# Decade-qiu/Go2NetSpectra

Measured on AMD Instinct MI355X. Metric: Mpackets/s CMS update (device-resident, d=4 w=2^20) at 1/2/4/8 MI355X, higher is better.
Workload: dtype u32; 1 GPU; configs[1]: Count-Min d=4 w=2^20, 100M Zipf(1.1) 5-tuple headers in HBM per GPU, bit-exact counters; device_batch=100000000, key=5-tuple (37 B), parallelism=owner-key shards x1 (SrcIP slot; each GPU generates its shard of the stream), windows=steps use stream windows 0..619 (warmup first), none replayed

## Files before the change

go2netspectra_amd/csrc/gns_cm.hip:

```cpp
#include <algorithm>
#include <atomic>
#include <cstdlib>
#include <mutex>
#include <vector>

#include "gns_coldmask.cuh"
#include "gns_common.hpp"
#include "gns_ctl.cuh"
#include "gns_hh.hpp"
#include "gns_scan.cuh"
#include "gns_xcd.cuh"

namespace gns {

#ifndef GNS_TILE_BITS
#define GNS_TILE_BITS 12
#endif
#ifndef GNS_AP_THREADS
#define GNS_AP_THREADS 1024
#endif
#ifndef GNS_AP_ITEMS
#define GNS_AP_ITEMS 8
#endif
constexpr uint32_t kTileBitsMax = GNS_TILE_BITS;
// ... 2294 lines not shown
        uint32_t cum = 0, t = kHotKeys;
        for (int k = (int)kHotKeys - 1; k >= (int)(kHotMinBits * 8); k--) {
            cum += s_hh[r * kHotKeys + k];
            if (cum > kHot) break;
            t = (uint32_t)k;
        }
        const uint32_t tp = thr[r];
        hfull[r] = !(tp <= kHotKeys && t + 8u >= tp && hcn[r] <= kHotCand);
        thr[r] = t;
        hcnt[r] = 0;
    }
}

__global__ __launch_bounds__(256) void k_hot_collect(const uint32_t *C, CmGeom g, const uint32_t *thr,
                                                      uint32_t *hcnt, uint32_t *hot_ids, const uint32_t *hcand,
                                                      const uint32_t *hcn, const uint32_t *hfull) {
    const uint64_t stride = (uint64_t)gridDim.x * 256;
    for (uint32_t r = 0; r < g.d; r++) {
        const uint32_t *Cr = C + (uint64_t)r * g.w;
        const uint32_t t = thr[r];
        auto take = [&](uint32_t v, uint64_t c) {
            if (v >= (1u << (kHotMinBits - 1)) && hot_key(v) >= t) {
                const uint32_t q = atomicAdd(&hcnt[r], 1u);
                if (q < kHot) hot_ids[r * kHot + q] = (uint32_t)c;
            }
        };
        if (!hfull[r]) {
            const uint32_t nc = hcn[r];
            for (uint32_t i = blockIdx.x * 256 + threadIdx.x; i < nc; i += (uint32_t)stride) {
                const uint32_t c = hcand[(uint64_t)r * kHotCand + i];
                take(Cr[c], c);
            }
            continue;
        }
        if ((g.w & 3u) == 0) {
            const uint4 *C4 = reinterpret_cast<const uint4 *>(Cr);
            for (uint64_t c = (uint64_t)blockIdx.x * 256 + threadIdx.x; c < g.w / 4; c += stride) {
                const uint4 v = C4[c];
                take(v.x, 4 * c); take(v.y, 4 * c + 1); take(v.z, 4 * c + 2); take(v.w, 4 * c + 3);
            }
        } else {
            for (uint64_t c = (uint64_t)blockIdx.x * 256 + threadIdx.x; c < g.w; c += stride) take(Cr[c], c);
        }
    }
}

__global__ __launch_bounds__(1024) void k_hot_table(CmGeom g, uint32_t *hot_ids, uint32_t *hot_tab, uint32_t *hcn) {
    __shared__ uint32_t s_ids[8 * kHot];
    const uint32_t NS = g.d * kHot;
    for (uint32_t i = threadIdx.x; i < g.d * kHotTab; i += blockDim.x) hot_tab[i] = 0xFFFFFFFFu;
    if (threadIdx.x < g.d) hcn[threadIdx.x] = 0;
    for (uint32_t i = threadIdx.x; i < NS; i += blockDim.x) s_ids[i] = hot_ids[i];
    __syncthreads();
    for (uint32_t i = threadIdx.x; i < NS; i += blockDim.x) {
        const uint32_t r = i / kHot, h = i % kHot, b = s_ids[i];
        if (b == GNS_ID_NONE) continue;
        const uint32_t grp = hot_group(b);
        uint32_t j = 0;
        for (uint32_t h2 = 0; h2 < h; h2++) {
            const uint32_t b2 = s_ids[r * kHot + h2];
            j += (b2 != GNS_ID_NONE && hot_group(b2) == grp) ? 1u : 0u;
        }
        if (j < 4) hot_tab[r * kHotTab + grp * 4 + j] = b << kHotBits | h;
        else hot_ids[i] = GNS_ID_NONE;
    }
}

struct QueryArgs {
    const uint8_t *keys;
    uint32_t stride, aligned;
    uint64_t n;
    uint32_t K;
    CmGeom g;
    DictDev D;
    const uint32_t *C, *Fc, *S, *Fs;
    uint64_t *out;
};

__global__ __launch_bounds__(256) void k_query(QueryArgs a) {
    const uint64_t p = (uint64_t)blockIdx.x * 256 + threadIdx.x;
    if (p >= a.n) return;
    uint32_t kw[GNS_KWMAX];
    load_key_bytes<GNS_KWMAX>(a.keys + p * a.stride, a.K, a.aligned != 0, kw);
    const uint32_t id = dict_lookup(a.D, kw);
    uint32_t sz = 0, ct = 0;
    if (id != GNS_ID_NONE) {
        for (uint32_t rr = 0; rr < a.g.d; rr++) {
            const uint64_t c = (uint64_t)rr * a.g.w + row_index(a.g, mm3_n<GNS_KWMAX>(kw, a.K, a.g.seeds[rr]));
            if (a.Fs[c] == id) sz = max(sz, a.S[c]);
            if (a.Fc[c] == id) ct = max(ct, a.C[c]);
        }
    }
    a.out[p] = (uint64_t)ct << 32 | sz;
}

}

using namespace gns;

struct CmRead {
    HhScratch hh;
    uint8_t *qkeys = nullptr;
    uint64_t qkeys_n = 0;
    uint64_t *qout = nullptr;
    uint64_t qout_n = 0;
    void free_all() {
        hh.free_all();
        dfree(qkeys); dfree(qout);
        qkeys = nullptr; qout = nullptr;
        qkeys_n = qout_n = 0;
    }
};

struct gns_cm : FlowDict {
    int device = 0;
    hipStream_t stream = nullptr;
    CmGeom g{};
    KeyPlanN kp{};
    uint32_t K = 0, st = 0, ct = 0;
    uint32_t *C = nullptr, *S = nullptr, *Fc = nullptr, *Fs = nullptr;
    CmRead rd;
    std::atomic<uint32_t> period{0};
    std::mutex views_mu;
    std::vector<gns_cm_view *> views;
    uint32_t epoch = 0;
    uint64_t bmax = 0;
    uint32_t nblk_max = 0;
    uint32_t *keyid = nullptr, *idx = nullptr;
    uint64_t *cold = nullptr;
    uint64_t *pend[2] = {nullptr, nullptr};
    uint32_t *pcnt[2] = {nullptr, nullptr};
    uint32_t *ptotal = nullptr;
    uint32_t *hist = nullptr, *part = nullptr, *total = nullptr, *order = nullptr;
    uint64_t *entries = nullptr;
    uint32_t *rec_sizes = nullptr;
    uint64_t *ovf = nullptr;
    uint32_t *ovf_cnt = nullptr;
    uint64_t ovf_cap = 0;
    unsigned long long *stats = nullptr;
    uint32_t *hot_ids = nullptr;
    uint32_t *hot_tab = nullptr;
    long long *segtot = nullptr;
    uint32_t *hflag = nullptr, *hhist = nullptr, *hthr = nullptr, *hcnt = nullptr;
    uint32_t *hcand = nullptr, *hcn = nullptr;
    HotSum *hsum = nullptr;
    uint32_t *hflag2 = nullptr;
    uint32_t *work = nullptr;
    uint32_t ncu = 256;
    uint32_t *hres = nullptr;
    uint4 *chk = nullptr;
    bool warm = false;
    bool lds_ordered = false;
    uint32_t *h_pin = nullptr;
    HostStage stage[2];
    uint32_t *side_dev = nullptr;
    uint64_t side_n = 0;
    hipStream_t cstream = nullptr;
    hipEvent_t ev_copied[2] = {nullptr, nullptr}, ev_used[2] = {nullptr, nullptr};
    StageTimer timer;
};

struct gns_cm_view {
    gns_cm *cm = nullptr;
    hipStream_t stream = nullptr;
    hipEvent_t ready = nullptr;
    uint32_t *C = nullptr, *S = nullptr, *Fc = nullptr, *Fs = nullptr;
    CmRead rd;
    std::mutex mu;
    uint32_t period = ~0u;
};

struct ViewsQuiesced {
    std::unique_lock<std::mutex> reg;
    std::vector<std::unique_lock<std::mutex>> locks;
    explicit ViewsQuiesced(gns_cm *cm) : reg(cm->views_mu) {
        locks.reserve(cm->views.size());
        for (gns_cm_view *v : cm->views) locks.emplace_back(v->mu);
    }
};

namespace {

int cm_free_all(gns_cm *cm) {
    dfree(cm->C); dfree(cm->S); dfree(cm->Fc); dfree(cm->Fs); cm->rd.free_all();
    dfree(cm->keyid); dfree(cm->idx); dfree(cm->cold);
    dfree(cm->pend[0]); dfree(cm->pend[1]); dfree(cm->pcnt[0]); dfree(cm->pcnt[1]);
    dfree(cm->ptotal); dfree(cm->hist); dfree(cm->part); dfree(cm->total); dfree(cm->order);
    dfree(cm->entries); dfree(cm->rec_sizes); dfree(cm->ovf); dfree(cm->ovf_cnt); dfree(cm->stats);
    cm->stage[0].free_all(); cm->stage[1].free_all(); dfree(cm->side_dev);
    for (int i = 0; i < 2; i++) {
        if (cm->ev_copied[i]) (void)hipEventDestroy(cm->ev_copied[i]);
        if (cm->ev_used[i]) (void)hipEventDestroy(cm->ev_used[i]);
    }
    if (cm->cstream) (void)hipStreamDestroy(cm->cstream);
    dfree(cm->work);
    dfree(cm->hot_ids); dfree(cm->segtot); dfree(cm->hflag); dfree(cm->hhist); dfree(cm->hthr); dfree(cm->hcnt);
    dfree(cm->hcand); dfree(cm->hcn);
    dfree(cm->hsum); dfree(cm->hflag2); dfree(cm->hres); dfree(cm->chk); dfree(cm->hot_tab);
    cm->FlowDict::free_all();
    if (cm->h_pin) (void)hipHostFree(cm->h_pin);
    cm->timer.destroy();
    if (cm->stream) (void)hipStreamDestroy(cm->stream);
    return GNS_OK;
}

int cm_reset_state(gns_cm *cm) {
    const uint64_t cells = (uint64_t)cm->g.d * cm->g.w;
    GNS_HIP(hipMemsetAsync(cm->C, 0, cells * 4, cm->stream));
    GNS_HIP(hipMemsetAsync(cm->S, 0, cells * 4, cm->stream));
    GNS_HIP(hipMemsetAsync(cm->Fc, 0xFF, cells * 4, cm->stream));
    GNS_HIP(hipMemsetAsync(cm->Fs, 0xFF, cells * 4, cm->stream));
    GNS_HIP(hipMemsetAsync(cm->D.rec, 0, cm->dict_slots * cm->D.RW * 4, cm->stream));
    GNS_HIP(hipMemsetAsync(cm->hot_ids, 0xFF, (size_t)cm->g.d * kHot * 4, cm->stream));
    GNS_HIP(hipMemsetAsync(cm->hot_tab, 0xFF, (size_t)cm->g.d * kHotTab * 4, cm->stream));
    GNS_HIP(hipMemsetAsync(cm->hhist, 0, (size_t)cm->g.d * kHotKeys * 4, cm->stream));
    GNS_HIP(hipMemsetAsync(cm->hthr, 0xFF, 8 * 4, cm->stream));
    GNS_HIP(hipMemsetAsync(cm->hcn, 0, 16 * 4, cm->stream));
    GNS_HIP(hipMemsetAsync(cm->stats + 3, 0, 2 * sizeof(unsigned long long), cm->stream));
    GNS_HIP(hipMemsetAsync(cm->dctl, 0, 16, cm->stream));
    cm->claimed = 0;
    cm->full = false;
    cm->warm = false;
    return GNS_OK;
}

int cm_reclaim(gns_cm *cm, uint64_t min_slots = 0) {
    ViewsQuiesced q(cm);
    const uint64_t cells = (uint64_t)cm->g.d * cm->g.w;
    std::vector<DictIds> ids{{cm->Fc, cells}, {cm->Fs, cells}};
    const uint32_t period = cm->period.load();
    for (gns_cm_view *v : cm->views)
        if (v->period == period) { ids.push_back({v->Fc, cells}); ids.push_back({v->Fs, cells}); }
    return cm->reclaim(ids.data(), (int)ids.size(), min_slots, cm->stream);
}

template <int KIND, int MODE>
int cm_run_batch(gns_cm *cm, const InputDesc &in, uint64_t n) {
    if (n == 0) return GNS_OK;
    hipStream_t s = cm->stream;
    const uint32_t nblk = (uint32_t)((n + kChunk - 1) / kChunk);
    const CmGeom &g = cm->g;
    ScopedStage total_stage(cm->timer, 5);
    {
        CtlZero z;
        z.add(cm->ptotal, 8);
        z.add(cm->dctl + 1, 4);
        z.add(cm->hflag2, ((size_t)g.d * kHot + 2) * 4);
        z.add(cm->stats + 8, 8);
        z.add(cm->ovf_cnt, 4);
        z.add(cm->work, 4);
        z.add(cm->hflag, (size_t)g.d * kHot * 4);
        GNS_HIP(ctl_zero(z, s));
    }
    if (++cm->epoch == 0) cm->epoch = 1;
    {
        ExtractArgs a{};
        a.in = in; a.n = n; a.kp = cm->kp; a.g = g; a.D = cm->D; a.epoch = cm->epoch;
        a.keyid = cm->keyid; a.idx = cm->idx; a.cold = cm->cold; a.pend = cm->pend[0]; a.pend_cnt = cm->pcnt[0];
        a.pend_total = cm->ptotal; a.hist = cm->hist; a.nblk = nblk; a.hot_ids = cm->hot_ids;
        a.Fc = cm->Fc; a.Fs = cm->Fs; a.hsum = cm->hsum; a.hot_tab = cm->hot_tab;
        a.stats = cm->stats;
        ScopedStage st(cm->timer, 0);
        const size_t lds = extract_lds_bytes(g.nbins_all, g.d);
        if constexpr (KIND == IN_REC16) {
            if (lds > kExLdsSmall)
                hipLaunchKernelGGL((k_extract<KIND, MODE, 0, 0, 1024>), dim3(nblk), dim3(1024), lds, s, a);
            else
                hipLaunchKernelGGL((k_extract<KIND, MODE, 0, 0, 256>), dim3(nblk), dim3(kExThreads), lds, s, a);
        } else if (lds > kExLdsSmall) {
            if (cm->K == 37 && g.d == 8)
                hipLaunchKernelGGL((k_extract<KIND, MODE, 37, 8, kC5Threads>), dim3(nblk), dim3(kC5Threads), lds, s, a);
            else if (cm->K == 37)
                hipLaunchKernelGGL((k_extract<KIND, MODE, 37, 0, 1024>), dim3(nblk), dim3(1024), lds, s, a);
            else if (cm->K == 16)
                hipLaunchKernelGGL((k_extract<KIND, MODE, 16, 0, 1024>), dim3(nblk), dim3(1024), lds, s, a);
            else
                hipLaunchKernelGGL((k_extract<KIND, MODE, 0, 0, 1024>), dim3(nblk), dim3(1024), lds, s, a);
        } else if (cm->K == 37 && g.d == 4)
            hipLaunchKernelGGL((k_extract<KIND, MODE, 37, 4, 256>), dim3(nblk), dim3(kExThreads), lds, s, a);
        else if (cm->K == 37)
            hipLaunchKernelGGL((k_extract<KIND, MODE, 37, 0, 256>), dim3(nblk), dim3(kExThreads), lds, s, a);
        else if (cm->K == 16 && g.d == 4)
            hipLaunchKernelGGL((k_extract<KIND, MODE, 16, 4, 256>), dim3(nblk), dim3(kExThreads), lds, s, a);
        else if (cm->K == 16)
            hipLaunchKernelGGL((k_extract<KIND, MODE, 16, 0, 256>), dim3(nblk), dim3(kExThreads), lds, s, a);
        else
            hipLaunchKernelGGL((k_extract<KIND, MODE, 0, 0, 256>), dim3(nblk), dim3(kExThreads), lds, s, a);
        GNS_HIP(hipGetLastError());
    }
    int cur = 0;
    for (int round = 0;; round++) {
        if (round > 1) {
            CtlRead rd;
            rd.add(cm->ptotal + cur, 4, 0);
            rd.add(cm->stats + 3, 8, 2);
            rd.add(cm->dctl, 4, 4);
            if (round == 2) rd.add(cm->stats + 8, 8, 6);
            GNS_HIP(ctl_read(rd, cm->h_pin, s));
            GNS_HIP(hipStreamSynchronize(s));
            cm->claimed = cm->h_pin[4];
            if (round == 2) {
                const uint64_t big = (uint64_t)cm->h_pin[6] | (uint64_t)cm->h_pin[7] << 32;
                if (big * g.d > cm->ovf_cap) {
                    const uint64_t want = std::min<uint64_t>(std::max<uint64_t>(big * g.d + big * g.d / 4, kOvfCap), 1ull << 31);
                    dfree(cm->ovf);
                    cm->ovf = nullptr;
                    cm->ovf_cap = 0;
                    GNS_TRY(dalloc_t(&cm->ovf, want));
                    cm->ovf_cap = want;
                }
            }
            if (cm->h_pin[2] | cm->h_pin[3]) {
                set_error("flow dictionary full (%llu slots); raise max_flows",
                          (unsigned long long)cm->dict_slots);
                return GNS_E_FULL;
            }
            if (cm->h_pin[0] == 0) break;
        }
        if (round > 64) { set_error("dictionary resolve did not converge"); return GNS_E_FULL; }
        if (++cm->epoch == 0) cm->epoch = 1;
        ResolveArgs a{};
        a.in = in; a.n = n; a.kp = cm->kp; a.D = cm->D; a.epoch = cm->epoch; a.keyid = cm->keyid;
        a.pend_in = cm->pend[cur]; a.cnt_in = cm->pcnt[cur];
        a.pend_out = cm->pend[cur ^ 1]; a.cnt_out = cm->pcnt[cur ^ 1]; a.total_out = cm->ptotal + (cur ^ 1);
        a.total_in = cm->ptotal + cur;
        a.stats = cm->stats; a.g = g;
        ScopedStage st(cm->timer, 1);
        hipLaunchKernelGGL((k_resolve<KIND, MODE>), dim3(nblk), dim3(kExThreads), 0, s, a);
        GNS_HIP(hipGetLastError());
        cur ^= 1;
    }
    {
        ScopedStage st(cm->timer, 2);
        const uint32_t ngrp = (nblk + kTGrp - 1) / kTGrp;
        const dim3 g2((g.nbins_all + 255) / 256, ngrp);
        uint32_t *tot = cm->part + (size_t)ngrp * g.nbins_all;
        hipLaunchKernelGGL(k_tscan_part, g2, dim3(256), 0, s, cm->hist, nblk, g.nbins_all, cm->part);
        hipLaunchKernelGGL(k_tscan_mid, dim3((g.nbins_all + 255) / 256), dim3(256), 0, s, cm->part, ngrp, g.nbins_all, tot);
        hipLaunchKernelGGL(k_tscan_bins, dim3(1), dim3(1024), 0, s, tot, g.nbins_all, cm->total);
        hipLaunchKernelGGL(k_tscan_down, g2, dim3(256), 0, s, cm->hist, nblk, g.nbins_all, cm->part, tot);
        GNS_HIP(hipGetLastError());
    }
    {
        ScatterArgs a{};
        a.n = n; a.g = g; a.keyid = cm->keyid; a.idx = cm->idx; a.sizes = in.sizes;
        a.offsets = cm->hist; a.nblk = nblk; a.entries = cm->entries; a.ovf = cm->ovf; a.cold = cm->cold;
        a.ovf_cnt = cm->ovf_cnt; a.ovf_cap = (uint32_t)cm->ovf_cap; a.hot_ids = cm->hot_ids; a.stats = cm->stats;
        a.hot_mode = 0; a.hflag2 = cm->hflag2; a.hany = cm->hflag2 + g.d * kHot;
        ScopedStage st(cm->timer, 3);
        if (cm->lds_ordered && g.ntiles <= 256)
            hipLaunchKernelGGL((k_scatter_st<256, false>), dim3(nblk), dim3(kStThreads), 0, s, a);
        else if (cm->lds_ordered && g.ntiles <= 512)
            hipLaunchKernelGGL((k_scatter_st<512, true>), dim3(nblk), dim3(kStThreads), 0, s, a);
        else if (cm->lds_ordered)
            hipLaunchKernelGGL(k_scatter<1>, dim3(nblk), dim3(kScThreads), scatter_lds_bytes(g.ntiles + kHot, g.d), s, a);
        else
            hipLaunchKernelGGL(k_scatter<0>, dim3(nblk), dim3(kScThreads), scatter_lds_bytes(g.ntiles + kHot, g.d), s, a);
        GNS_HIP(hipGetLastError());
    }
    {
        const bool ordered = g.nbins <= 4096;
        if (ordered)
            hipLaunchKernelGGL(k_order, dim3(1), dim3(1024), 0, s, cm->hist, nblk, g.nbins, g.nbins_all,
                               cm->total, cm->order);
        ApplyArgs a{};
        a.stats = cm->stats;
        a.entries = cm->entries; a.offsets = cm->hist; a.nblk = nblk; a.nbins = g.nbins;
        a.total = cm->total; a.order = ordered ? cm->order : nullptr; a.ovf = cm->ovf; a.g = g;
        a.C = cm->C; a.Fc = cm->Fc; a.S = cm->S; a.Fs = cm->Fs; a.work = cm->work;
        ScopedStage st(cm->timer, 4);
        if (g.sub_bits) {
            const dim3 apg(std::min(g.nbins, cm->ncu));
            hipLaunchKernelGGL(k_apply_sparse, apg, dim3(kApThreads), 0, s, a);
        } else {
            const dim3 apg(std::min(g.nbins, cm->ncu * (kApThreads <= 512 ? 2u : 1u)));
            hipLaunchKernelGGL(k_apply, apg, dim3(kApThreads), 0, s, a);
        }
        GNS_HIP(hipGetLastError());
    }
    {
        HotArgs h{};
        h.entries = cm->entries; h.offsets = cm->hist; h.nblk = nblk; h.total = cm->total; h.ovf = cm->ovf;
        h.hot_ids = cm->hot_ids; h.g = g; h.C = cm->C; h.Fc = cm->Fc; h.S = cm->S; h.Fs = cm->Fs;
        h.segtot = cm->segtot; h.hflag = cm->hflag;
        h.hsum = cm->hsum; h.hflag2 = cm->hflag2; h.hany = cm->hflag2 + g.d * kHot; h.nchk = h.hany + 1;
        h.hres = cm->hres; h.chk = cm->chk; h.chk_cap = kChkCap;
        h.keyid = cm->keyid; h.idx = cm->idx; h.sizes = in.sizes; h.n = n;
        ScopedStage st(cm->timer, 6);
        hipLaunchKernelGGL(k_hot_decide, dim3(g.d * kHot), dim3(256), 0, s, h);
        hipLaunchKernelGGL(k_hot_blockcheck, dim3(kChkCap), dim3(256), 0, s, h);
        hipLaunchKernelGGL(k_hot_commit, dim3((g.d * kHot + 511) / 512), dim3(512), 0, s, h);
        {
            ScatterArgs a{};
            a.n = n; a.g = g; a.keyid = cm->keyid; a.idx = cm->idx; a.sizes = in.sizes;
            a.offsets = cm->hist; a.nblk = nblk; a.entries = cm->entries; a.ovf = cm->ovf;
            a.ovf_cnt = cm->ovf_cnt; a.ovf_cap = (uint32_t)cm->ovf_cap; a.hot_ids = cm->hot_ids; a.stats = cm->stats;
            a.hot_mode = 1; a.hflag2 = cm->hflag2; a.hany = h.hany;
            if (cm->lds_ordered)
                hipLaunchKernelGGL(k_scatter<1>, dim3(nblk), dim3(kScThreads), scatter_lds_bytes(g.ntiles + kHot, g.d), s, a);
            else
                hipLaunchKernelGGL(k_scatter<0>, dim3(nblk), dim3(kScThreads), scatter_lds_bytes(g.ntiles + kHot, g.d), s, a);
        }
        hipLaunchKernelGGL(k_hot_sum, dim3(1024), dim3(256), 0, s, h);
        hipLaunchKernelGGL(k_hot_verify, dim3(1024), dim3(256), 0, s, h);
        hipLaunchKernelGGL(k_hot_apply, dim3((g.d * kHot + 511) / 512), dim3(512), 0, s, h);
        hipLaunchKernelGGL(k_hot_fallback, dim3(g.d * kHot), dim3(64), 0, s, h);
        GNS_HIP(hipGetLastError());
    }
    {
        ScopedStage st(cm->timer, 7);
        const unsigned grid = (unsigned)std::min<uint64_t>(2048, ((uint64_t)g.w / 4 + 255) / 256 + 1);
        uint32_t *hcn = cm->hcn, *hfull = cm->hcn + 8;
        hipLaunchKernelGGL(k_hot_hist, dim3(std::min(grid, 512u)), dim3(256), 0, s, cm->C, g, cm->hhist, cm->hthr,
                           cm->hcand, hcn);
        hipLaunchKernelGGL(k_hot_pick, dim3(1), dim3(512), 0, s, cm->hhist, g, cm->hthr, cm->hcnt, cm->hot_ids, hcn,
                           hfull);
        hipLaunchKernelGGL(k_hot_collect, dim3(grid), dim3(256), 0, s, cm->C, g, cm->hthr, cm->hcnt, cm->hot_ids,
                           cm->hcand, hcn, hfull);
        hipLaunchKernelGGL(k_hot_table, dim3(1), dim3(1024), 0, s, g, cm->hot_ids, cm->hot_tab, hcn);
        GNS_HIP(hipGetLastError());
    }
    cm->warm = true;
    return GNS_OK;
}

template <int KIND>
int cm_batch(gns_cm *cm, const InputDesc &d, uint64_t m) {
    if constexpr (KIND == IN_KEYS) {
        return cm_run_batch<KIND, PLAN_SLICE0>(cm, d, m);
    } else {
        switch (plan_mode(cm->kp)) {
        case PLAN_SLICE0: return cm_run_batch<KIND, PLAN_SLICE0>(cm, d, m);
        case PLAN_SLICE4: return cm_run_batch<KIND, PLAN_SLICE4>(cm, d, m);
        default: return cm_run_batch<KIND, PLAN_GENERIC>(cm, d, m);
        }
    }
}

template <int KIND>
int cm_batch_recover(gns_cm *cm, const InputDesc &d, uint64_t m) {
    static const std::string piece = std::to_string(kChunk) + "-packet batch";
    const DictRecovery r{*cm, cm->stats, cm->stream, kChunk, piece.c_str(),
                         [cm](const InputDesc &pd, uint64_t pm) { return cm_batch<KIND>(cm, pd, pm); },
                         [cm](uint64_t min_slots) { return cm_reclaim(cm, min_slots); }};
    return r.batch(d, m, false);
}

__global__ __launch_bounds__(256) void k_rec_sizes(const uint32_t *rec16, uint64_t n, uint32_t *sizes) {
    const uint64_t i = (uint64_t)blockIdx.x * 256 + threadIdx.x;
    if (i < n) sizes[i] = rec16[i * 4 + 3] >> 16;
}

int stage_host_batch(gns_cm *cm, int b, const InputDesc &in, uint64_t off, uint64_t m, InputDesc &d) {
    if (!cm->cstream) {
        GNS_HIP(hipStreamCreateWithFlags(&cm->cstream, hipStreamNonBlocking));
        for (int i = 0; i < 2; i++) {
            GNS_HIP(hipEventCreateWithFlags(&cm->ev_copied[i], hipEventDisableTiming));
            GNS_HIP(hipEventCreateWithFlags(&cm->ev_used[i], hipEventDisableTiming));
        }
    }
    StageList l;
    d = advance(in, off);
    stage_input(l, d, m);
    if (in.rec_len) stage_add<uint32_t>(l, nullptr, m * 4, &d.sizes);
    HostStage &sg = cm->stage[b];
    if (sg.cap < HostStage::need(l)) GNS_HIP(hipEventSynchronize(cm->ev_used[b]));
    GNS_HIP(hipStreamWaitEvent(cm->cstream, cm->ev_used[b], 0));
    GNS_TRY(sg.copy(l, cm->cstream));
    if (in.rec_len) {
        hipLaunchKernelGGL(k_rec_sizes, dim3((unsigned)((m + 255) / 256)), dim3(256), 0, cm->cstream, d.rec16, m,
                           const_cast<uint32_t *>(d.sizes));
        GNS_HIP(hipGetLastError());
    }
    if (d.keys) d.aligned = (d.stride % 4 == 0 && d.stride >= ((cm->K + 3) & ~3u)) ? 1u : 0u;
    GNS_HIP(hipEventRecord(cm->ev_copied[b], cm->cstream));
    return GNS_OK;
}

template <int KIND>
int cm_insert(gns_cm *cm, InputDesc in, uint64_t n, gns_mem where) {
    GNS_TRY(set_device(cm->device));
    auto batch_len = [&](uint64_t off, bool warm) {
        const uint64_t m = std::min<uint64_t>(cm->bmax, n - off);
        return warm ? m : std::min<uint64_t>(m, std::max<uint64_t>(kChunk * 64, cm->bmax / 32));
    };
    if (where == GNS_MEM_DEVICE) {
        for (uint64_t off = 0, m = 0; off < n; off += m) {
            m = batch_len(off, cm->warm);
            InputDesc d = advance(in, off);
            if (in.rec_len) {
                if (!cm->rec_sizes) GNS_TRY(dalloc_t(&cm->rec_sizes, cm->bmax));
                hipLaunchKernelGGL(k_rec_sizes, dim3((unsigned)((m + 255) / 256)), dim3(256), 0, cm->stream, d.rec16, m,
                                   cm->rec_sizes);
                GNS_HIP(hipGetLastError());
                d.sizes = cm->rec_sizes;
            }
            GNS_TRY(cm_batch_recover<KIND>(cm, d, m));
        }
        return GNS_OK;
    }
    if (n == 0) return GNS_OK;
    bool warm = cm->warm;
    uint64_t off = 0, m = batch_len(0, warm);
    InputDesc d;
    GNS_TRY(stage_host_batch(cm, 0, in, 0, m, d));
    for (int b = 0;; b ^= 1) {
        const uint64_t noff = off + m;
        const uint64_t nm = noff < n ? batch_len(noff, true) : 0;
        InputDesc nd;
        if (nm) GNS_TRY(stage_host_batch(cm, b ^ 1, in, noff, nm, nd));
        GNS_HIP(hipStreamWaitEvent(cm->stream, cm->ev_copied[b], 0));
        const int rc = cm_batch_recover<KIND>(cm, d, m);
        GNS_HIP(hipEventRecord(cm->ev_used[b], cm->stream));
        if (rc != GNS_OK) {
            (void)hipStreamSynchronize(cm->cstream);
            return rc;
        }
        if (!nm) break;
        off = noff; m = nm; d = nd;
    }
    GNS_HIP(hipStreamSynchronize(cm->cstream));
    return GNS_OK;
}

}

extern "C" {

int gns_cm_create(const gns_cm_params *p, gns_cm **out) {
    if (!p || !out) { set_error("null argument"); return GNS_E_ARG; }
    *out = nullptr;
    GNS_TRY(check_device(p->device));
    gns_cm *cm = new gns_cm();
    cm->device = p->device;
    int rc = GNS_OK;
    do {
        if ((rc = set_device(cm->device)) != GNS_OK) break;
        CmGeom &g = cm->g;
        g.w = p->width ? p->width : (1u << 20);
        g.d = p->depth ? p->depth : 3u;
        cm->st = p->size_threshold ? p->size_threshold : 512u * 1024u;
        cm->ct = p->count_threshold ? p->count_threshold : 512u;
        if (g.d > 8) { set_error("depth %u > 8 not supported", g.d); rc = GNS_E_ARG; break; }
        if ((rc = make_plan(p->flow, p->key_bytes, &cm->kp)) != GNS_OK) break;
        cm->K = cm->kp.K;
        if (g.w >= (1u << (32 - kHotBits))) {
            set_error("width %u >= 2^%u is not supported", g.w, 32 - kHotBits); rc = GNS_E_RANGE; break;
        }
        if (p->bucket_lo == 0 && p->bucket_hi == 0) {
            g.blo = 0; g.bspan = g.w;
        } else if (p->bucket_lo < p->bucket_hi && p->bucket_hi <= g.w) {
            g.blo = p->bucket_lo; g.bspan = p->bucket_hi - p->bucket_lo;
        } else {
            set_error("bucket range [%u, %u) is not inside [0, %u)", p->bucket_lo, p->bucket_hi, g.w);
            rc = GNS_E_ARG; break;
        }
        g.pow2 = (g.w & (g.w - 1)) == 0;
        g.wmask = g.pow2 ? g.w - 1 : 0;
        uint32_t tb = kTileBitsMax;
        while (tb > 8 && (uint64_t)g.d * ((g.w + (1u << tb) - 1) >> tb) < 1024) tb--;
        g.tile_bits = tb;
        uint32_t sb = 0;
        auto bins_at = [&](uint32_t bits) { return (uint32_t)(((uint64_t)g.w + (1ull << bits) - 1) >> bits); };
        while (bins_at(tb + sb) > kMaxTilesPerRow || (uint64_t)g.d * bins_at(tb + sb) > kMaxBinsAll) sb++;
        if (tb + sb > kEntShift || sb > 4) {
            set_error("width %u with depth %u is too wide (max %u buckets per row at this depth)", g.w, g.d,
                      (uint32_t)std::min<uint64_t>(0xFFFFFFFFull, (uint64_t)std::min(kMaxTilesPerRow, kMaxBinsAll / g.d) << kEntShift));
            rc = GNS_E_RANGE;
            break;
        }
        g.sub_bits = sb;
        g.bin_bits = tb + sb;
        g.ntiles = bins_at(g.bin_bits);
        g.nbins = g.d * g.ntiles;
        g.nbins_all = g.nbins + g.d * kHot;
        g.nbits = ceil_log2(g.ntiles + kHot);
        if (p->seeds) for (uint32_t i = 0; i < g.d; i++) g.seeds[i] = p->seeds[i];
        else default_seeds(g.seeds, g.d);
        if (hipStreamCreateWithFlags(&cm->stream, hipStreamNonBlocking) != hipSuccess) {
            set_error("hipStreamCreate failed"); rc = GNS_E_HIP; break;
        }
        cm->timer.stream = cm->stream;
        {
            int ncu = 0;
            if (hipDeviceGetAttribute(&ncu, hipDeviceAttributeMultiprocessorCount, cm->device) == hipSuccess && ncu > 0)
                cm->ncu = (uint32_t)ncu;
        }
        const uint64_t cells = (uint64_t)g.d * g.w;
        if ((rc = dalloc_t(&cm->C, cells)) || (rc = dalloc_t(&cm->S, cells)) ||
            (rc = dalloc_t(&cm->Fc, cells)) || (rc = dalloc_t(&cm->Fs, cells)))
            break;
        const uint64_t mf = p->max_flows ? p->max_flows : (4ull << 20);
        uint64_t slots = 1;
        while (slots < 2 * mf) slots <<= 1;
        if (slots > kDictMaxSlots) { set_error("max_flows too large"); rc = GNS_E_ARG; break; }
        cm->dict_slots = slots;
        cm->max_flows = mf;
        cm->D.mask = (uint32_t)(slots - 1);
        cm->D.K = cm->K;
        cm->D.RW = dict_record_words_cm(cm->K, g.d);
        cm->D.bw = cm->D.RW >= 16 && 1 + (cm->K + 3) / 4 <= 12 ? 1u : 0u;
        cm->D.seed = 0x2545F491u;
        if ((rc = dalloc_t(&cm->D.rec, slots * cm->D.RW)) != GNS_OK) break;
        if ((rc = dalloc_t(&cm->dctl, 4)) != GNS_OK || (rc = dalloc_t(&cm->stats_bak, 3)) != GNS_OK) break;
        cm->D.ctl = cm->dctl;
        cm->limits();
        cm->bmax = p->batch_packets ? p->batch_packets : (16ull << 20);
        cm->bmax = ((cm->bmax + kChunk - 1) / kChunk) * kChunk;
        if (cm->bmax > (1ull << 31)) { set_error("batch_packets too large"); rc = GNS_E_ARG; break; }
        const uint64_t bcap = (((1ull << 31) / g.d) / kChunk) * kChunk;
        if (cm->bmax > bcap) cm->bmax = bcap;
        cm->nblk_max = (uint32_t)(cm->bmax / kChunk);
        const uint64_t nscan = ((uint64_t)(cm->nblk_max + kTGrp - 1) / kTGrp + 2) * g.nbins_all;
        if ((rc = dalloc_t(&cm->keyid, cm->bmax)) || (rc = dalloc_t(&cm->idx, cm->bmax * g.d)) ||
            (rc = dalloc_t(&cm->cold, cm->bmax / 64)) ||
            (rc = dalloc_t(&cm->pend[0], cm->bmax)) || (rc = dalloc_t(&cm->pend[1], cm->bmax)) ||
            (rc = dalloc_t(&cm->pcnt[0], cm->nblk_max)) || (rc = dalloc_t(&cm->pcnt[1], cm->nblk_max)) ||
            (rc = dalloc_t(&cm->ptotal, 2)) || (rc = dalloc_t(&cm->hist, (uint64_t)g.nbins_all * cm->nblk_max)) ||
            (rc = dalloc_t(&cm->part, nscan)) || (rc = dalloc_t(&cm->total, 1)) ||
            (rc = dalloc_t(&cm->order, g.nbins)) || (rc = dalloc_t(&cm->entries, cm->bmax * g.d)) ||
            (rc = dalloc_t(&cm->ovf, kOvfCap)) || (rc = dalloc_t(&cm->ovf_cnt, 1)) ||
            (rc = dalloc_t(&cm->stats, kStatsProf + 16)) || (rc = dalloc_t(&cm->work, 1)) || (rc = dalloc_t(&cm->hot_ids, g.d * kHot)) ||
            (rc = dalloc_t(&cm->segtot, (size_t)g.d * kHot * kHotSegs * 2)) || (rc = dalloc_t(&cm->hflag, g.d * kHot)) ||
            (rc = dalloc_t(&cm->hhist, g.d * kHotKeys)) || (rc = dalloc_t(&cm->hthr, 8)) || (rc = dalloc_t(&cm->hcnt, 8)) ||
            (rc = dalloc_t(&cm->hcand, (size_t)g.d * kHotCand)) || (rc = dalloc_t(&cm->hcn, 16)) ||
            (rc = dalloc_t(&cm->hsum, (uint64_t)g.d * kHot * cm->nblk_max)) ||
            (rc = dalloc_t(&cm->hflag2, g.d * kHot + 2)) || (rc = dalloc_t(&cm->hres, g.d * kHot * 2)) ||
            (rc = dalloc_t(&cm->chk, kChkCap)) || (rc = dalloc_t(&cm->hot_tab, (size_t)g.d * kHotTab)))
            break;
        cm->ovf_cap = kOvfCap;
        if (hipHostMalloc(reinterpret_cast<void **>(&cm->h_pin), 64, 0) != hipSuccess) {
            set_error("hipHostMalloc failed"); rc = GNS_E_OOM; break;
        }
        if (hipMemsetAsync(cm->stats, 0, (kStatsProf + 16) * 8, cm->stream) != hipSuccess) { rc = GNS_E_HIP; break; }
        if ((rc = cm_reset_state(cm)) != GNS_OK) break;
        {
            const char *env = getenv("GNS_K3_RANK");
            uint32_t *viol = nullptr;
            if ((rc = dalloc_t(&viol, 1)) != GNS_OK) break;
            hipError_t e = hipMemsetAsync(viol, 0, 4, cm->stream);
            if (e == hipSuccess) {
                hipLaunchKernelGGL(k_lds_order_probe, dim3(4 * cm->ncu), dim3(256), 0, cm->stream, viol, 64);
                e = hipGetLastError();
            }
            uint32_t hv = 1;
            if (e == hipSuccess) e = hipMemcpyAsync(&hv, viol, 4, hipMemcpyDeviceToHost, cm->stream);
            if (e == hipSuccess) e = hipStreamSynchronize(cm->stream);
            dfree(viol);
            if (e != hipSuccess) { set_error("lds order probe: %s", hipGetErrorString(e)); rc = GNS_E_HIP; break; }
            cm->lds_ordered = hv == 0 && !(env && env[0] == '0');
        }
        if ((rc = hh_reserve(cm->rd.hh, (uint64_t)cm->g.d * cm->g.w, cm->dict_slots, cm->K, cm->stream)) != GNS_OK) break;
        if (hipStreamSynchronize(cm->stream) != hipSuccess) { set_error("sync failed"); rc = GNS_E_HIP; break; }
    } while (0);
    if (rc != GNS_OK) {
        cm_free_all(cm);
        delete cm;
        return rc;
    }
    *out = cm;
    return GNS_OK;
}

int gns_cm_destroy(gns_cm *cm) {
    if (!cm) return GNS_OK;
    (void)hipSetDevice(cm->device);
    if (cm->stream) (void)hipStreamSynchronize(cm->stream);
    cm_free_all(cm);
    delete cm;
    return GNS_OK;
}

int gns_cm_insert_keys(gns_cm *cm, const uint8_t *keys, uint32_t stride, const uint32_t *sizes,
                       uint64_t n, gns_mem where) {
    if (!cm || (n && (!keys || !sizes))) { set_error("null argument"); return GNS_E_ARG; }
    if (stride < cm->K) { set_error("stride %u < key_bytes %u", stride, cm->K); return GNS_E_ARG; }
    InputDesc in{};
    in.keys = keys; in.stride = stride; in.sizes = sizes;
    in.aligned = (stride % 4 == 0 && (reinterpret_cast<uintptr_t>(keys) & 3) == 0 &&
                  stride >= ((cm->K + 3) & ~3u)) ? 1u : 0u;
    return cm_insert<IN_KEYS>(cm, in, n, where);
}

int gns_cm_insert_tuples(gns_cm *cm, const gns_tuples *t, uint64_t n, gns_mem where) {
    if (!cm || !t) { set_error("null argument"); return GNS_E_ARG; }
    if (n && (!t->src16 || !t->dst16 || !t->sport || !t->dport || !t->proto || !t->length)) {
        set_error("null tuple array"); return GNS_E_ARG;
    }
    InputDesc in{};
    in.src16 = t->src16; in.dst16 = t->dst16; in.sport = t->sport; in.dport = t->dport;
    in.proto = t->proto; in.sizes = t->length;
    return cm_insert<IN_TUPLE>(cm, in, n, where);
}

int gns_cm_insert_headers(gns_cm *cm, const uint8_t *hdr, const uint32_t *wirelen, uint64_t n,
                          gns_mem where) {
    if (!cm || (n && (!hdr || !wirelen))) { set_error("null argument"); return GNS_E_ARG; }
    InputDesc in{};
    in.hdr = reinterpret_cast<const uint32_t *>(hdr);
    in.sizes = wirelen;
    return cm_insert<IN_HDR>(cm, in, n, where);
}

int gns_cm_insert_compact(gns_cm *cm, const uint8_t *rec16, const uint32_t *wirelen, uint64_t n,
                          const uint8_t *side64, uint64_t n_side, gns_mem where) {
    if (!cm || (n && !rec16) || (n_side && !side64)) { set_error("null argument"); return GNS_E_ARG; }
    InputDesc in{};
    in.rec16 = reinterpret_cast<const uint32_t *>(rec16);
    in.sizes = wirelen;
    in.rec_len = wirelen ? 0u : 1u;
    in.side = reinterpret_cast<const uint32_t *>(side64);
    in.n_side = side64 ? n_side : 0;
    if (where == GNS_MEM_HOST && n_side) {
        GNS_TRY(set_device(cm->device));
        GNS_HIP(hipStreamSynchronize(cm->stream));
        if (cm->side_n < n_side) {
            dfree(cm->side_dev);
            cm->side_dev = nullptr;
            cm->side_n = 0;
            GNS_TRY(dalloc_t(&cm->side_dev, n_side * 16));
            cm->side_n = n_side;
        }
        GNS_HIP(hipMemcpy(cm->side_dev, side64, n_side * 64, hipMemcpyHostToDevice));
        in.side = cm->side_dev;
    }
    return cm_insert<IN_REC16>(cm, in, n, where);
}

int gns_cm_flush(gns_cm *cm) {
    if (!cm) return GNS_E_ARG;
    GNS_TRY(set_device(cm->device));
    {
        CtlRead rd;
        rd.add(cm->stats + 4, 48, 0);
        GNS_HIP(ctl_read(rd, cm->h_pin, cm->stream));
    }
    GNS_HIP(hipStreamSynchronize(cm->stream));
    cm->timer.collect();
    if (cm->h_pin[0] | cm->h_pin[1]) {
        set_error("overflow side table exhausted (internal error)");
        return GNS_E_RANGE;
    }
    if (cm->h_pin[10] | cm->h_pin[11]) {
        set_error("sparse K4: an update's bucket was not in its table (internal error)");
        return GNS_E_HIP;
    }
    return GNS_OK;
}

}

static int cm_query_impl(gns_cm *cm, hipStream_t st, CmRead &sc, const uint32_t *C, const uint32_t *Fc,
                         const uint32_t *S, const uint32_t *Fs, const uint8_t *keys, uint32_t stride, uint64_t n,
                         uint64_t *out, bool dev = false) {
    if (!dev) {
        GNS_TRY(grow_buf(&sc.qkeys, sc.qkeys_n, n * stride));
        GNS_TRY(grow_buf(&sc.qout, sc.qout_n, n));
    }
    QueryArgs a{};
    a.keys = dev ? keys : sc.qkeys;
    a.stride = stride;
    a.aligned = (stride % 4 == 0 && stride >= ((cm->K + 3) & ~3u) && ((uintptr_t)a.keys & 3u) == 0);
    a.n = n; a.K = cm->K; a.g = cm->g; a.D = cm->D;
    a.C = C; a.Fc = Fc; a.S = S; a.Fs = Fs; a.out = dev ? out : sc.qout;
    hipError_t e = dev ? hipSuccess : hipMemcpyAsync(sc.qkeys, keys, n * stride, hipMemcpyHostToDevice, st);
    if (e == hipSuccess) {
        hipLaunchKernelGGL(k_query, dim3((unsigned)((n + 255) / 256)), dim3(256), 0, st, a);
        e = hipGetLastError();
    }
    if (e == hipSuccess && !dev) e = hipMemcpyAsync(out, sc.qout, n * 8, hipMemcpyDeviceToHost, st);
    if (e == hipSuccess) e = hipStreamSynchronize(st);
    if (e != hipSuccess) { set_error("query: %s", hipGetErrorString(e)); return GNS_E_HIP; }
    return GNS_OK;
}

extern "C" {

int gns_cm_query(gns_cm *cm, const uint8_t *keys, uint32_t stride, uint64_t n, uint64_t *out) {
    if (!cm || (n && (!keys || !out))) { set_error("null argument"); return GNS_E_ARG; }
    if (n == 0) return GNS_OK;
    if (stride < cm->K) { set_error("stride < key_bytes"); return GNS_E_ARG; }
    GNS_TRY(set_device(cm->device));
    return cm_query_impl(cm, cm->stream, cm->rd, cm->C, cm->Fc, cm->S, cm->Fs, keys, stride, n, out);
}

int gns_cm_query_device(gns_cm *cm, const uint8_t *keys, uint32_t stride, uint64_t n, uint64_t *out) {
// ... 314 lines not shown
```

Before: 22680 Mpackets/s.

## Overlap resolve control readback with scan and skip idle hot-key passes

Restructures the host-device control flow of the CMS update. The first control readback is now recorded with an event, so the tally scan, order and hot-decide kernels are queued before the host waits, which hides the round-trip latency. The readback also fetches the hot-key flags, so blockcheck is launched only with the needed grid size and the hot rescatter/apply is skipped when no hot keys need it. This adds more host/device ordering logic and some risk around the overflow buffer being reallocated after kernels that reference it have already been queued.

```diff
diff --git a/go2netspectra_amd/csrc/gns_cm.hip b/go2netspectra_amd/csrc/gns_cm.hip
--- a/go2netspectra_amd/csrc/gns_cm.hip
+++ b/go2netspectra_amd/csrc/gns_cm.hip
@@ -2470,6 +2470,7 @@
     bool warm = false;
     bool lds_ordered = false;
     uint32_t *h_pin = nullptr;
+    hipEvent_t ev_ctl = nullptr;
     HostStage stage[2];
     uint32_t *side_dev = nullptr;
     uint64_t side_n = 0;
@@ -2517,6 +2518,7 @@
     dfree(cm->hsum); dfree(cm->hflag2); dfree(cm->hres); dfree(cm->chk); dfree(cm->hot_tab);
     cm->FlowDict::free_all();
     if (cm->h_pin) (void)hipHostFree(cm->h_pin);
+    if (cm->ev_ctl) (void)hipEventDestroy(cm->ev_ctl);
     cm->timer.destroy();
     if (cm->stream) (void)hipStreamDestroy(cm->stream);
     return GNS_OK;
@@ -2607,35 +2609,7 @@
         GNS_HIP(hipGetLastError());
     }
     int cur = 0;
-    for (int round = 0;; round++) {
-        if (round > 1) {
-            CtlRead rd;
-            rd.add(cm->ptotal + cur, 4, 0);
-            rd.add(cm->stats + 3, 8, 2);
-            rd.add(cm->dctl, 4, 4);
-            if (round == 2) rd.add(cm->stats + 8, 8, 6);
-            GNS_HIP(ctl_read(rd, cm->h_pin, s));
-            GNS_HIP(hipStreamSynchronize(s));
-            cm->claimed = cm->h_pin[4];
-            if (round == 2) {
-                const uint64_t big = (uint64_t)cm->h_pin[6] | (uint64_t)cm->h_pin[7] << 32;
-                if (big * g.d > cm->ovf_cap) {
-                    const uint64_t want = std::min<uint64_t>(std::max<uint64_t>(big * g.d + big * g.d / 4, kOvfCap), 1ull << 31);
-                    dfree(cm->ovf);
-                    cm->ovf = nullptr;
-                    cm->ovf_cap = 0;
-                    GNS_TRY(dalloc_t(&cm->ovf, want));
-                    cm->ovf_cap = want;
-                }
-            }
-            if (cm->h_pin[2] | cm->h_pin[3]) {
-                set_error("flow dictionary full (%llu slots); raise max_flows",
-                          (unsigned long long)cm->dict_slots);
-                return GNS_E_FULL;
-            }
-            if (cm->h_pin[0] == 0) break;
-        }
-        if (round > 64) { set_error("dictionary resolve did not converge"); return GNS_E_FULL; }
+    auto resolve_round = [&]() -> int {
         if (++cm->epoch == 0) cm->epoch = 1;
         ResolveArgs a{};
         a.in = in; a.n = n; a.kp = cm->kp; a.D = cm->D; a.epoch = cm->epoch; a.keyid = cm->keyid;
@@ -2647,6 +2621,31 @@
         hipLaunchKernelGGL((k_resolve<KIND, MODE>), dim3(nblk), dim3(kExThreads), 0, s, a);
         GNS_HIP(hipGetLastError());
         cur ^= 1;
+        return GNS_OK;
+    };
+    GNS_TRY(resolve_round());
+    GNS_TRY(resolve_round());
+    HotArgs h{};
+    h.entries = cm->entries; h.offsets = cm->hist; h.nblk = nblk; h.total = cm->total; h.ovf = cm->ovf;
+    h.hot_ids = cm->hot_ids; h.g = g; h.C = cm->C; h.Fc = cm->Fc; h.S = cm->S; h.Fs = cm->Fs;
+    h.segtot = cm->segtot; h.hflag = cm->hflag;
+    h.hsum = cm->hsum; h.hflag2 = cm->hflag2; h.hany = cm->hflag2 + g.d * kHot; h.nchk = h.hany + 1;
+    h.hres = cm->hres; h.chk = cm->chk; h.chk_cap = kChkCap;
+    h.keyid = cm->keyid; h.idx = cm->idx; h.sizes = in.sizes; h.n = n;
+    {
+        ScopedStage st(cm->timer, 6);
+        hipLaunchKernelGGL(k_hot_decide, dim3(g.d * kHot), dim3(256), 0, s, h);
+        GNS_HIP(hipGetLastError());
+    }
+    {
+        CtlRead rd;
+        rd.add(cm->ptotal + cur, 4, 0);
+        rd.add(cm->stats + 3, 8, 2);
+        rd.add(cm->dctl, 4, 4);
+        rd.add(cm->stats + 8, 8, 6);
+        rd.add(h.hany, 8, 8);
+        GNS_HIP(ctl_read(rd, cm->h_pin, s));
+        GNS_HIP(hipEventRecord(cm->ev_ctl, s));
     }
     {
         ScopedStage st(cm->timer, 2);
@@ -2658,6 +2657,57 @@
         hipLaunchKernelGGL(k_tscan_bins, dim3(1), dim3(1024), 0, s, tot, g.nbins_all, cm->total);
         hipLaunchKernelGGL(k_tscan_down, g2, dim3(256), 0, s, cm->hist, nblk, g.nbins_all, cm->part, tot);
         GNS_HIP(hipGetLastError());
+    }
+    const bool ordered = g.nbins <= 4096;
+    if (ordered) {
+        hipLaunchKernelGGL(k_order, dim3(1), dim3(1024), 0, s, cm->hist, nblk, g.nbins, g.nbins_all,
+                           cm->total, cm->order);
+        GNS_HIP(hipGetLastError());
+    }
+    uint32_t hany = 0, nchk = 0;
+    for (int round = 2;; round++) {
+        GNS_HIP(hipEventSynchronize(cm->ev_ctl));
+        cm->claimed = cm->h_pin[4];
+        if (round == 2) {
+            hany = cm->h_pin[8];
+            nchk = std::min<uint32_t>(cm->h_pin[9], kChkCap);
+            const uint64_t big = (uint64_t)cm->h_pin[6] | (uint64_t)cm->h_pin[7] << 32;
+            if (big * g.d > cm->ovf_cap) {
+                const uint64_t want = std::min<uint64_t>(std::max<uint64_t>(big * g.d + big * g.d / 4, kOvfCap), 1ull << 31);
+                dfree(cm->ovf);
+                cm->ovf = nullptr;
+                cm->ovf_cap = 0;
+                GNS_TRY(dalloc_t(&cm->ovf, want));
+                cm->ovf_cap = want;
+                h.ovf = cm->ovf;
+            }
+        }
+        if (cm->h_pin[2] | cm->h_pin[3]) {
+            set_error("flow dictionary full (%llu slots); raise max_flows",
+                      (unsigned long long)cm->dict_slots);
+            return GNS_E_FULL;
+        }
+        if (cm->h_pin[0] == 0) break;
+        if (round > 64) { set_error("dictionary resolve did not converge"); return GNS_E_FULL; }
+        GNS_TRY(resolve_round());
+        CtlRead rd;
+        rd.add(cm->ptotal + cur, 4, 0);
+        rd.add(cm->stats + 3, 8, 2);
+        rd.add(cm->dctl, 4, 4);
+        GNS_HIP(ctl_read(rd, cm->h_pin, s));
+        GNS_HIP(hipEventRecord(cm->ev_ctl, s));
+    }
+    {
+        ScopedStage st(cm->timer, 6);
+        if (nchk) hipLaunchKernelGGL(k_hot_blockcheck, dim3(nchk), dim3(256), 0, s, h);
+        hipLaunchKernelGGL(k_hot_commit, dim3((g.d * kHot + 511) / 512), dim3(512), 0, s, h);
+        GNS_HIP(hipGetLastError());
+    }
+    if (nchk) {
+        CtlRead rd;
+        rd.add(h.hany, 4, 8);
+        GNS_HIP(ctl_read(rd, cm->h_pin, s));
+        GNS_HIP(hipEventRecord(cm->ev_ctl, s));
     }
     {
         ScatterArgs a{};
@@ -2677,10 +2727,6 @@
         GNS_HIP(hipGetLastError());
     }
     {
-        const bool ordered = g.nbins <= 4096;
-        if (ordered)
-            hipLaunchKernelGGL(k_order, dim3(1), dim3(1024), 0, s, cm->hist, nblk, g.nbins, g.nbins_all,
-                               cm->total, cm->order);
         ApplyArgs a{};
         a.stats = cm->stats;
         a.entries = cm->entries; a.offsets = cm->hist; a.nblk = nblk; a.nbins = g.nbins;
@@ -2696,18 +2742,12 @@
         }
         GNS_HIP(hipGetLastError());
     }
-    {
-        HotArgs h{};
-        h.entries = cm->entries; h.offsets = cm->hist; h.nblk = nblk; h.total = cm->total; h.ovf = cm->ovf;
-        h.hot_ids = cm->hot_ids; h.g = g; h.C = cm->C; h.Fc = cm->Fc; h.S = cm->S; h.Fs = cm->Fs;
-        h.segtot = cm->segtot; h.hflag = cm->hflag;
-        h.hsum = cm->hsum; h.hflag2 = cm->hflag2; h.hany = cm->hflag2 + g.d * kHot; h.nchk = h.hany + 1;
-        h.hres = cm->hres; h.chk = cm->chk; h.chk_cap = kChkCap;
-        h.keyid = cm->keyid; h.idx = cm->idx; h.sizes = in.sizes; h.n = n;
+    if (nchk) {
+        GNS_HIP(hipEventSynchronize(cm->ev_ctl));
+        hany = cm->h_pin[8];
+    }
+    if (hany) {
         ScopedStage st(cm->timer, 6);
-        hipLaunchKernelGGL(k_hot_decide, dim3(g.d * kHot), dim3(256), 0, s, h);
-        hipLaunchKernelGGL(k_hot_blockcheck, dim3(kChkCap), dim3(256), 0, s, h);
-        hipLaunchKernelGGL(k_hot_commit, dim3((g.d * kHot + 511) / 512), dim3(512), 0, s, h);
         {
             ScatterArgs a{};
             a.n = n; a.g = g; a.keyid = cm->keyid; a.idx = cm->idx; a.sizes = in.sizes;
@@ -2950,6 +2990,9 @@
         if (hipHostMalloc(reinterpret_cast<void **>(&cm->h_pin), 64, 0) != hipSuccess) {
             set_error("hipHostMalloc failed"); rc = GNS_E_OOM; break;
         }
+        if (hipEventCreateWithFlags(&cm->ev_ctl, hipEventDisableTiming) != hipSuccess) {
+            set_error("hipEventCreate failed"); rc = GNS_E_HIP; break;
+        }
         if (hipMemsetAsync(cm->stats, 0, (kStatsProf + 16) * 8, cm->stream) != hipSuccess) { rc = GNS_E_HIP; break; }
         if ((rc = cm_reset_state(cm)) != GNS_OK) break;
         {
```

Measured after the change: 22760 Mpackets/s (median of 4 runs). No clear change (+0.3%).
